# jabberjabberjabber/video-3d-pipeline

Measured on AMD Instinct MI355X. Metric: 1080p_sbs_to_4k_depth_frames_per_s, higher is better.
Workload: dtype int16 (SGM) + f64 (guided filter sums; f32 depth in/out)

## Files before the change

### video-3d-pipeline_amd/csrc/v3d_guided.hip

```cpp
#include "v3d_common.h"
#include <type_traits>

__device__ __forceinline__ double gf_rcp(double x)
{
    double r = __builtin_amdgcn_rcp(x);
    r = fma(r, fma(-x, r, 1.0), r);
    r = fma(r, fma(-x, r, 1.0), r);
    return r;
}

template <typename TD> __device__ __forceinline__ float gf_ld(const TD* p, size_t i);
template <> __device__ __forceinline__ float gf_ld<float>(const float* p, size_t i) { const float v = p[i]; return fabsf(v) <= 3.402823466e38f ? v : 0.f; }
template <> __device__ __forceinline__ float gf_ld<int16_t>(const int16_t* p, size_t i) { const int d = p[i]; return d > 0 ? (float)d * 0.0625f : 0.f; }
template <> __device__ __forceinline__ float gf_ld<uint16_t>(const uint16_t* p, size_t i) { return (float)p[i]; }

typedef unsigned short v3d_u16x2v __attribute__((ext_vector_type(2)));
typedef unsigned short v3d_u16x4 __attribute__((ext_vector_type(4)));
__device__ __forceinline__ void gf_st(float* p, float q) { *p = q; }
__device__ __forceinline__ void gf_st(uint16_t* p, float q) { *p = v3d_rint_u16(q); }

#define GF_TX 64
#define GF_RUN 8
#define GF_RMAX 16

template <typename TD>
__device__ __forceinline__ double gf_bilinear(const TD* __restrict__ src, int Ws, int Hs, double sx, double sy, int x, int y)
{
    const double fx = (x + 0.5) * sx - 0.5, fy = (y + 0.5) * sy - 0.5;
    const double x0f = floor(fx), y0f = floor(fy);
    const double wx = fx - x0f, wy = fy - y0f;
    const int x0 = (int)x0f, y0 = (int)y0f;
    const int xa = min(max(x0, 0), Ws - 1), xb = min(max(x0 + 1, 0), Ws - 1);
    const int ya = min(max(y0, 0), Hs - 1), yb = min(max(y0 + 1, 0), Hs - 1);
    const double top = (double)gf_ld(src, (size_t)ya * Ws + xa) * (1.0 - wx) + (double)gf_ld(src, (size_t)ya * Ws + xb) * wx;
    const double bot = (double)gf_ld(src, (size_t)yb * Ws + xa) * (1.0 - wx) + (double)gf_ld(src, (size_t)yb * Ws + xb) * wx;
    return top * (1.0 - wy) + bot * wy;
}

template <int SWEEP, int GF_RUNY, typename TD, typename TO>
__global__ __launch_bounds__(256) void k_gf(const TD* __restrict__ depth_lo, int Wlo, int Hlo,
                                            const uint8_t* __restrict__ guide, int W, int H, int r, double eps,
                                            double* __restrict__ A, double* __restrict__ B, TO* __restrict__ out)
{
    constexpr int NS = SWEEP == 1 ? 4 : 2;
    constexpr int GF_TY = 4 * GF_RUNY;
    extern __shared__ __attribute__((aligned(16))) double smem[];
    const int rows = GF_TY + 2 * r;
    const int pitch = (GF_TX + 2 * r) | 1;
    const int hp = GF_TX + 1;
    double* t0 = smem;
    double* t1 = t0 + rows * pitch;
    double* hs = t1 + rows * pitch;

    const int tid = threadIdx.x;
    const int ox = blockIdx.x * GF_TX, oy = blockIdx.y * GF_TY;
    const double sx = (double)Wlo / (double)W, sy = (double)Hlo / (double)H;

    const int tw = GF_TX + 2 * r;
    for (int i = tid; i < rows * tw; i += 256) {
        const int ty = i / tw, tx = i - ty * tw;
        const int gx = ox - r + tx, gy = oy - r + ty;
        double v0 = 0.0, v1 = 0.0;
        if (gx >= 0 && gx < W && gy >= 0 && gy < H) {
            if (SWEEP == 1) {
                v0 = (double)guide[(size_t)gy * W + gx] / 255.0;
                v1 = gf_bilinear(depth_lo, Wlo, Hlo, sx, sy, gx, gy);
            } else {
                v0 = A[(size_t)gy * W + gx];
                v1 = B[(size_t)gy * W + gx];
            }
        }
        t0[ty * pitch + tx] = v0;
        t1[ty * pitch + tx] = v1;
    }
    __syncthreads();

    const int nruns = GF_TX / GF_RUN;
    for (int task = tid; task < rows * nruns; task += 256) {
        const int row = task % rows, run = task / rows;
        const double* r0 = t0 + row * pitch + run * GF_RUN;
        const double* r1 = t1 + row * pitch + run * GF_RUN;
        double s0 = 0.0, s1 = 0.0, s2 = 0.0, s3 = 0.0;
        for (int k = 0; k <= 2 * r; k++) {
            const double u = r0[k], v = r1[k];
            s0 += u; s1 += v;
            if (SWEEP == 1) { s2 += u * u; s3 += u * v; }
        }
        double* h = hs + row * hp + run * GF_RUN;
        const int hplane = rows * hp;
        for (int j = 0; j < GF_RUN; j++) {
            h[j] = s0; h[hplane + j] = s1;
            if (SWEEP == 1) { h[2 * hplane + j] = s2; h[3 * hplane + j] = s3; }
            if (j + 1 < GF_RUN) {
                const double un = r0[j + 2 * r + 1], vn = r1[j + 2 * r + 1];
                const double uo = r0[j], vo = r1[j];
                s0 += un - uo; s1 += vn - vo;
                if (SWEEP == 1) { s2 += un * un - uo * uo; s3 += un * vn - uo * vo; }
            }
        }
    }
    __syncthreads();

    {
        const int x = tid % GF_TX, runy = tid / GF_TX;
        const int hplane = rows * hp;
        const double* h = hs + (runy * GF_RUNY) * hp + x;
        double s[NS];
#pragma unroll
        for (int q = 0; q < NS; q++) s[q] = 0.0;
        for (int k = 0; k <= 2 * r; k++)
#pragma unroll
            for (int q = 0; q < NS; q++) s[q] += h[q * hplane + k * hp];
        const int gx = ox + x;
        const int cx = min(gx + r, W - 1) - max(gx - r, 0) + 1;
        for (int j = 0; j < GF_RUNY; j++) {
            const int gy = oy + runy * GF_RUNY + j;
            if (gx < W && gy < H) {
                const int cy = min(gy + r, H - 1) - max(gy - r, 0) + 1;
                const double cnt = (double)(cx * cy);
                if (SWEEP == 1) {
                    const double mI = s[0] / cnt, mp = s[1] / cnt, mII = s[2] / cnt, mIp = s[3] / cnt;
                    const double var = mII - mI * mI, cov = mIp - mI * mp;
                    const double a = cov / (var + eps);
                    A[(size_t)gy * W + gx] = a;
                    B[(size_t)gy * W + gx] = mp - a * mI;
                } else {
                    const double I = (double)guide[(size_t)gy * W + gx] / 255.0;
                    const float q = (float)((s[0] / cnt) * I + (s[1] / cnt));
                    if constexpr (std::is_same<TO, float>::value) out[(size_t)gy * W + gx] = q;
                    else out[(size_t)gy * W + gx] = v3d_rint_u16(q);
                }
            }
            if (j + 1 < GF_RUNY) {
                const int kn = j + 2 * r + 1;
#pragma unroll
                for (int q = 0; q < NS; q++) s[q] += h[q * hplane + kn * hp] - h[q * hplane + j * hp];
            }
        }
    }
}

#ifndef GF_CH
#define GF_CH 3
#endif
typedef double v3d_f64x2 __attribute__((ext_vector_type(2)));
typedef float v3d_f32x2 __attribute__((ext_vector_type(2)));
typedef float v3d_f32x4 __attribute__((ext_vector_type(4)));

template <int SWEEP, int RR, typename TD, typename TO>
__global__ __launch_bounds__(256) void k_gfm(const TD* __restrict__ depth_lo, int Wlo, int Hlo,
                                             const uint8_t* __restrict__ guide, int W, int H, double eps, int band_h,
                                             double* __restrict__ A, double* __restrict__ B, TO* __restrict__ out,
                                             size_t depth_stride, size_t guide_stride)
{
    static_assert(RR % 2 == 0, "pairs must not straddle the strip's halo boundary");
    constexpr int R = 2 * RR + 1, NOUT = 256 - 2 * RR;
    __shared__ __attribute__((aligned(16))) double sVd[2][2][2][256];
    __shared__ __attribute__((aligned(16))) int2 sVi[2][2][256];
    {
        const size_t f = blockIdx.z, n4 = (size_t)W * H;
        depth_lo += f * depth_stride; guide += f * guide_stride; A += f * 2 * n4; B += f * 2 * n4; out += f * n4;
    }
    const int tid = threadIdx.x;
    const int gx = blockIdx.x * NOUT - RR + tid;
    const int ya = blockIdx.y * band_h, yb = min(ya + band_h, H);
    const bool col_ok = gx >= 0 && gx < W;
    const double sx = (double)Wlo / (double)W, sy = (double)Hlo / (double)H;
    const int nsteps = (yb - ya) + 2 * RR;

    const int hrow = tid >> 7, hq = tid & 127;
    const int hgx = blockIdx.x * NOUT - RR + 2 * hq;
    const bool pair_in = 2 * hq >= RR && 2 * hq < 256 - RR;
    const bool px0 = pair_in && hgx < W, px1 = pair_in && hgx + 1 < W;
    const bool vec_ok = px1 && (W & 1) == 0;

    int bxa = 0, bxb = 0; double bwx = 0.0;
    if (SWEEP == 1) {
        const double fx = (gx + 0.5) * sx - 0.5, x0f = floor(fx);
        bwx = fx - x0f;
        bxa = min(max((int)x0f, 0), Wlo - 1); bxb = min(max((int)x0f + 1, 0), Wlo - 1);
    }
    double r0[R], r1[R], v0 = 0.0, v1 = 0.0;
    int rg[R], vg = 0, vgg = 0;
#pragma unroll
    for (int j = 0; j < R; j++) { r0[j] = 0.0; r1[j] = 0.0; rg[j] = 0; }

    struct RowIn { int g; float a0, a1, b0, b1; double n0, n1; bool in; };
    const int gxc = min(max(gx, 0), W - 1);
    auto fetch_row = [&](int t) -> RowIn {
        RowIn q; q.g = 0; q.a0 = q.a1 = q.b0 = q.b1 = 0.f; q.n0 = q.n1 = 0.0;
        const int e = ya - RR + t;
        q.in = col_ok && e >= 0 && e < H && t < nsteps;
        const size_t o = (size_t)min(max(e, 0), H - 1) * W + gxc;
        if (SWEEP == 1) {
            q.g = guide[o];
            const double fy = (e + 0.5) * sy - 0.5, y0f = floor(fy);
            const TD* ra = depth_lo + (size_t)min(max((int)y0f, 0), Hlo - 1) * Wlo;
            const TD* rb = depth_lo + (size_t)min(max((int)y0f + 1, 0), Hlo - 1) * Wlo;
            q.a0 = gf_ld(ra, bxa); q.a1 = gf_ld(ra, bxb); q.b0 = gf_ld(rb, bxa); q.b1 = gf_ld(rb, bxb);
        } else {
            q.n0 = __builtin_nontemporal_load(A + o); q.n1 = __builtin_nontemporal_load(B + o);
        }
        return q;
    };
    RowIn nx[2] = { fetch_row(0), fetch_row(1) };

    int buf = 0;
    for (int t0 = 0; t0 < nsteps; t0 += 2 * R) {
#pragma unroll
        for (int s = 0; s < R; s++) {
            const int tA = t0 + 2 * s;
            if (tA < nsteps) {
                const int y0 = ya - 2 * RR + tA;
                const bool emit = y0 >= ya;
                const RowIn cur[2] = { nx[0], nx[1] };
                nx[0] = fetch_row(tA + 2); nx[1] = fetch_row(tA + 3);
#pragma unroll
                for (int rr = 0; rr < 2; rr++) {
                    const int j = (2 * s + rr) % R;
                    if (SWEEP == 1) {
                        int gn = 0; double pn = 0.0;
                        if (cur[rr].in) {
                            gn = cur[rr].g;
                            const int e = ya - RR + tA + rr;
                            const double fy = (e + 0.5) * sy - 0.5, wy = fy - floor(fy);
                            const double a0 = (double)cur[rr].a0, b0 = (double)cur[rr].b0;
                            const double top = fma(bwx, (double)cur[rr].a1 - a0, a0);
                            const double bot = fma(bwx, (double)cur[rr].b1 - b0, b0);
                            pn = fma(wy, bot - top, top);
                        }
                        const int go = rg[j]; const double po = r1[j];
                        rg[j] = gn; r1[j] = pn;
                        vg += gn - go; vgg += gn * gn - go * go;
                        v0 += pn - po; v1 = fma((double)gn, pn, fma(-(double)go, po, v1));
                    } else {
                        const double n0 = cur[rr].in ? cur[rr].n0 : 0.0, n1 = cur[rr].in ? cur[rr].n1 : 0.0;
                        const double o0 = r0[j], o1 = r1[j];
                        r0[j] = n0; r1[j] = n1;
                        v0 += n0 - o0; v1 += n1 - o1;
                    }
                    if (emit) {
                        sVd[buf][rr][0][tid] = v0; sVd[buf][rr][1][tid] = v1;
                        if (SWEEP == 1) sVi[buf][rr][tid] = make_int2(vg, vgg);
                    }
                }
                if (emit) {
                    __syncthreads();
                    const int y = y0 + hrow;
                    if (px0 && y < yb) {
                        double fq[2], lq[2], cq[2];
#pragma unroll
                        for (int q = 0; q < 2; q++) {
                            const v3d_f64x2* d = reinterpret_cast<const v3d_f64x2*>(&sVd[buf][hrow][q][0]) + (hq - RR / 2);
                            double f = 0.0, l = 0.0, c = 0.0;
#pragma unroll
                            for (int ch = 0; ch <= RR; ch += GF_CH) {
                                v3d_f64x2 w[GF_CH];
#pragma unroll
                                for (int i = 0; i < GF_CH; i++) if (ch + i <= RR) w[i] = d[ch + i];
#pragma unroll
                                for (int i = 0; i < GF_CH; i++) if (ch + i <= RR) {
                                    if (ch + i == 0) { f = w[i].x; c = w[i].y; }
                                    else if (ch + i == RR) { c += w[i].x; l = w[i].y; }
                                    else { c += w[i].x; c += w[i].y; }
                                }
                                asm volatile("" : "+v"(c) :: "memory");
                            }
                            fq[q] = f; lq[q] = l; cq[q] = c;
                        }
                        int g0 = 0, gg0 = 0, gl = 0, ggl = 0, cg = 0, cgg = 0;
                        if (SWEEP == 1) {
                            const int4* gi = reinterpret_cast<const int4*>(&sVi[buf][hrow][0]) + (hq - RR / 2);
#pragma unroll
                            for (int ch = 0; ch <= RR; ch += 3) {
                                int4 u[3];
#pragma unroll
                                for (int i = 0; i < 3; i++) if (ch + i <= RR) u[i] = gi[ch + i];
#pragma unroll
                                for (int i = 0; i < 3; i++) if (ch + i <= RR) {
                                    if (ch + i == 0) { g0 = u[i].x; gg0 = u[i].y; cg = u[i].z; cgg = u[i].w; }
                                    else if (ch + i == RR) { cg += u[i].x; cgg += u[i].y; gl = u[i].z; ggl = u[i].w; }
                                    else { cg += u[i].x + u[i].z; cgg += u[i].y + u[i].w; }
                                }
                                asm volatile("" : "+v"(cg), "+v"(cgg) :: "memory");
                            }
                        }
                        const double s0a = cq[0] + fq[0], s0b = cq[0] + lq[0], s1a = cq[1] + fq[1], s1b = cq[1] + lq[1];
                        const int cy = min(y + RR, H - 1) - max(y - RR, 0) + 1;
                        const int cx0 = min(hgx + RR, W - 1) - max(hgx - RR, 0) + 1, cx1 = min(hgx + 1 + RR, W - 1) - max(hgx + 1 - RR, 0) + 1;
                        const double inva = gf_rcp((double)(cx0 * cy)), invb = cx1 == cx0 ? inva : gf_rcp((double)(cx1 * cy));
                        const size_t o = (size_t)y * W + hgx;
                        if (SWEEP == 1) {
                            const int sga = cg + g0, sgb = cg + gl, sgga = cgg + gg0, sggb = cgg + ggl;
                            double ab[2][2];
#pragma unroll
                            for (int n = 0; n < 2; n++) {
                                const double inv = n ? invb : inva;
                                const double mI = (double)(n ? sgb : sga) * (inv * (1.0 / 255.0)), mp = (n ? s0b : s0a) * inv;
                                const double mII = (double)(n ? sggb : sgga) * (inv * (1.0 / 65025.0)), mIp = (n ? s1b : s1a) * (inv * (1.0 / 255.0));
                                const double var = fma(-mI, mI, mII), cov = fma(-mI, mp, mIp);
                                const double a = cov * gf_rcp(var + eps);
                                ab[n][0] = a; ab[n][1] = fma(-a, mI, mp);
                            }
                            if (vec_ok) {
                                v3d_f64x2 va = { ab[0][0], ab[1][0] }, vb = { ab[0][1], ab[1][1] };
                                __builtin_nontemporal_store(va, reinterpret_cast<v3d_f64x2*>(A + o));
                                __builtin_nontemporal_store(vb, reinterpret_cast<v3d_f64x2*>(B + o));
                            } else {
                                A[o] = ab[0][0]; B[o] = ab[0][1];
                                if (px1) { A[o + 1] = ab[1][0]; B[o + 1] = ab[1][1]; }
                            }
                        } else {
                            const double Ia = (double)guide[o] * (1.0 / 255.0);
                            const double Ib = px1 ? (double)guide[o + 1] * (1.0 / 255.0) : 0.0;
                            const float qa = (float)((s0a * inva) * Ia + (s1a * inva)), qb = (float)((s0b * invb) * Ib + (s1b * invb));
                            if (vec_ok && (std::is_same<TO, float>::value || (reinterpret_cast<uintptr_t>(out + o) & 3) == 0)) {
                                if constexpr (std::is_same<TO, float>::value) {
                                    v3d_f32x2 vq = { qa, qb };
                                    __builtin_nontemporal_store(vq, reinterpret_cast<v3d_f32x2*>(out + o));
                                } else {
                                    v3d_u16x2v vq = { v3d_rint_u16(qa), v3d_rint_u16(qb) };
                                    __builtin_nontemporal_store(vq, reinterpret_cast<v3d_u16x2v*>(out + o));
                                }
                            } else {
                                gf_st(out + o, qa);
                                if (px1) gf_st(out + o + 1, qb);
                            }
                        }
                    }
                    buf ^= 1;
                }
            }
        }
    }
}

__device__ __forceinline__ int gf_swz2(int m) { return m ^ ((m >> 3) & 1) ^ ((m >> 4) & 1); }
__device__ __forceinline__ int gf_swz4(int m) { return m ^ ((m >> 4) & 3); }
__device__ __forceinline__ int gf_c8(int c) { return 2 * gf_swz2(c >> 1) + (c & 1); }

template <int RR>
__device__ __forceinline__ void gf_run4(const double* row, int c0, double s[4])
{
    const v3d_f64x2* d = reinterpret_cast<const v3d_f64x2*>(row);
    const int m0 = (c0 - RR) >> 1;
    double c = 0.0, l0 = 0.0, l1 = 0.0, l2 = 0.0, r1 = 0.0, r2 = 0.0, r3 = 0.0;
#pragma unroll
    for (int k0 = 0; k0 < RR + 2; k0 += GF_CH) {
        v3d_f64x2 w[GF_CH];
#pragma unroll
        for (int i = 0; i < GF_CH; i++) if (k0 + i < RR + 2) w[i] = d[gf_swz2(m0 + k0 + i)];
#pragma unroll
        for (int i = 0; i < GF_CH; i++) {
            const int k = k0 + i;
            if (k == 0) { l0 = w[i].x; l1 = w[i].y; c = w[i].x; c += w[i].y; }
            else if (k == 1) { l2 = w[i].x; c += w[i].x; c += w[i].y; }
            else if (k < RR) { c += w[i].x; c += w[i].y; }
            else if (k == RR) { c += w[i].x; r1 = w[i].y; }
            else if (k == RR + 1) { r2 = w[i].x; r3 = w[i].y; }
        }
        asm volatile("" : "+v"(c) :: "memory");
    }
    s[0] = c; s[1] = (s[0] + r1) - l0; s[2] = (s[1] + r2) - l1; s[3] = (s[2] + r3) - l2;
}

template <int RR>
__device__ __forceinline__ void gf_run4(const int2* row, int c0, int2 s[4])
{
    const int4* d = reinterpret_cast<const int4*>(row);
    const int m0 = (c0 - RR) >> 1;
    int2 c = make_int2(0, 0), l0 = c, l1 = c, l2 = c, r1 = c, r2 = c, r3 = c;
#pragma unroll
    for (int k0 = 0; k0 < RR + 2; k0 += 3) {
        int4 w[3];
#pragma unroll
        for (int i = 0; i < 3; i++) if (k0 + i < RR + 2) w[i] = d[gf_swz2(m0 + k0 + i)];
#pragma unroll
        for (int i = 0; i < 3; i++) {
            const int k = k0 + i;
            const int2 a = make_int2(w[i].x, w[i].y), b = make_int2(w[i].z, w[i].w);
            if (k == 0) { l0 = a; l1 = b; c = make_int2(a.x + b.x, a.y + b.y); }
            else if (k == 1) { l2 = a; c.x += a.x + b.x; c.y += a.y + b.y; }
            else if (k < RR) { c.x += a.x + b.x; c.y += a.y + b.y; }
            else if (k == RR) { c.x += a.x; c.y += a.y; r1 = b; }
            else if (k == RR + 1) { r2 = a; r3 = b; }
        }
        asm volatile("" : "+v"(c.x), "+v"(c.y) :: "memory");
    }
    s[0] = c;
    s[1] = make_int2(s[0].x + r1.x - l0.x, s[0].y + r1.y - l0.y);
    s[2] = make_int2(s[1].x + r2.x - l1.x, s[1].y + r2.y - l1.y);
    s[3] = make_int2(s[2].x + r3.x - l2.x, s[2].y + r3.y - l2.y);
}

template <int RR>
__device__ __forceinline__ void gf_run4(const int4* row, int c0, int4 s[4])
{
    int4 c = make_int4(0, 0, 0, 0), l0 = c, l1 = c, l2 = c, r1 = c, r2 = c, r3 = c;
#pragma unroll
    for (int k0 = 0; k0 < 2 * RR + 4; k0 += 3) {
        int4 u[3];
#pragma unroll
        for (int i = 0; i < 3; i++) if (k0 + i < 2 * RR + 4) u[i] = row[gf_swz4(c0 - RR + k0 + i)];
#pragma unroll
        for (int i = 0; i < 3; i++) {
            const int k = k0 + i;
            if (k < 2 * RR + 1) { c.x += u[i].x; c.y += u[i].y; c.z += u[i].z; c.w += u[i].w; }
            if (k == 0) l0 = u[i];
            else if (k == 1) l1 = u[i];
            else if (k == 2) l2 = u[i];
            else if (k == 2 * RR + 1) r1 = u[i];
            else if (k == 2 * RR + 2) r2 = u[i];
            else if (k == 2 * RR + 3) r3 = u[i];
        }
        asm volatile("" : "+v"(c.x), "+v"(c.y), "+v"(c.z), "+v"(c.w) :: "memory");
    }
    s[0] = c;
    s[1] = make_int4(s[0].x - l0.x + r1.x, s[0].y - l0.y + r1.y, s[0].z - l0.z + r1.z, s[0].w - l0.w + r1.w);
    s[2] = make_int4(s[1].x - l1.x + r2.x, s[1].y - l1.y + r2.y, s[1].z - l1.z + r2.z, s[1].w - l1.w + r2.w);
    s[3] = make_int4(s[2].x - l2.x + r3.x, s[2].y - l2.y + r3.y, s[2].z - l2.z + r3.z, s[2].w - l2.w + r3.w);
}

template <int RR>
__device__ __forceinline__ void gf_solve4(const int sg[4], const int sgg[4], const double sp[4], const double sgp[4], int hgx, int y,
                                          int W, int H, double eps, double a[4], double b[4])
{
    const int cy = min(y + RR, H - 1) - max(y - RR, 0) + 1;
    int cx[4];
#pragma unroll
    for (int n = 0; n < 4; n++) cx[n] = min(hgx + n + RR, W - 1) - max(hgx + n - RR, 0) + 1;
    const double inv0 = gf_rcp((double)(cx[0] * cy));
#pragma unroll
    for (int n = 0; n < 4; n++) {
        const double inv = (n == 0 || cx[n] == cx[0]) ? inv0 : gf_rcp((double)(cx[n] * cy));
        const double mI = (double)sg[n] * (inv * (1.0 / 255.0)), mp = sp[n] * inv;
        const double mII = (double)sgg[n] * (inv * (1.0 / 65025.0)), mIp = sgp[n] * (inv * (1.0 / 255.0));
        const double var = fma(-mI, mI, mII), cov = fma(-mI, mp, mIp);
        const double aa = cov * gf_rcp(var + eps);
        a[n] = aa; b[n] = fma(-aa, mI, mp);
    }
}

template <int RR, int COLS, typename TD, bool I1, typename TO>
__global__ __launch_bounds__(2 * COLS, I1 ? 4 : 2) void k_gff(const TD* __restrict__ depth_lo, int Wlo, int Hlo,
                                                const uint8_t* __restrict__ guide, int W, int H, double eps, int band_h,
                                                TO* __restrict__ out, size_t depth_stride, size_t guide_stride)
{
    static_assert(RR % 4 == 0, "runs of four must not straddle the strip's halo boundaries");
    static_assert(!I1 || std::is_same<TD, int16_t>::value, "the integer stage 1 takes the int16 disparity");
    static_assert(COLS == 256 || (COLS == 512 && I1), "strip width (512 columns: I1 only, the f64 route's rows exceed the LDS)");
    constexpr int R = 2 * RR + 1, NOUT = COLS - 4 * RR, HR = COLS / 4;
    constexpr int S1D = 2 * 4 * 2 * COLS * 8, S1 = I1 ? 2 * 4 * COLS * 16 : S1D + 2 * 4 * COLS * 8;
    __shared__ __attribute__((aligned(16))) unsigned char sS1[S1];
    double (*sV1)[4][2][COLS] = reinterpret_cast<double (*)[4][2][COLS]>(sS1);
    int2 (*sVi)[4][COLS] = reinterpret_cast<int2 (*)[4][COLS]>(sS1 + (I1 ? 0 : S1D));
    int4 (*sVq)[4][COLS] = reinterpret_cast<int4 (*)[4][COLS]>(sS1);
    (void)sV1; (void)sVi; (void)sVq;
    __shared__ __attribute__((aligned(16))) double sAB[3][4][2][COLS];
    {
        const size_t f = blockIdx.z, n4 = (size_t)W * H;
        depth_lo += f * depth_stride; guide += f * guide_stride; out += f * n4;
    }
    const int role = __builtin_amdgcn_readfirstlane((int)(threadIdx.x / COLS));
    const int t = threadIdx.x % COLS;
    const int gx0 = blockIdx.x * NOUT - 2 * RR;
    const int gx = gx0 + t;
    const int ya = blockIdx.y * band_h, yb = min(ya + band_h, H);
    const int nrows = (yb - ya) + 4 * RR;
    const int NS = (nrows + 3) >> 2;
    const int NP = NS + 3;

    if (role == 0) {
        const bool col_ok = gx >= 0 && gx < W;
        const int gxc = min(max(gx, 0), W - 1);
        uint32_t ring[R];
        double r1[I1 ? 1 : R];
        uint32_t rgw[I1 ? 1 : (R + 3) / 4];
        int vg = 0, vgg = 0, vP = 0, vgP = 0;
        double v0 = 0.0, v1 = 0.0;
#pragma unroll
        for (int j = 0; j < R; j++) ring[j] = 0u;
#pragma unroll
        for (int j = 0; j < (I1 ? 1 : R); j++) r1[j] = 0.0;
#pragma unroll
        for (int j = 0; j < (I1 ? 1 : (R + 3) / 4); j++) rgw[j] = 0u;
        (void)ring; (void)r1; (void)rgw;
        int bxa, bxb, wxa = 0, wxb = 0; double bwx = 0.0;
        const double sx = (double)Wlo / (double)W, sy = (double)Hlo / (double)H;
        if constexpr (I1) {
            const int kx = gx >> 1;
            bxa = min(max((gx & 1) ? kx : kx - 1, 0), Wlo - 1); bxb = min(max((gx & 1) ? kx + 1 : kx, 0), Wlo - 1);
            wxa = (gx & 1) ? 3 : 1; wxb = 4 - wxa;
        } else {
            const double fx = (gx + 0.5) * sx - 0.5, x0f = floor(fx);
            bwx = fx - x0f;
            bxa = min(max((int)x0f, 0), Wlo - 1); bxb = min(max((int)x0f + 1, 0), Wlo - 1);
        }
        (void)wxa; (void)wxb; (void)bwx;
        struct RowIn { int g; typename std::conditional<I1, int, float>::type a0, a1, b0, b1; bool in; };
        auto fetch_row = [&](int tt) -> RowIn {
            RowIn q;
            const int e = ya - 2 * RR + tt;
            q.in = col_ok && e >= 0 && e < H && tt < nrows;
            const int ec = min(max(e, 0), H - 1);
            q.g = guide[(size_t)ec * W + gxc];
            if constexpr (I1) {
                const int ky = ec >> 1;
                const TD* ra = depth_lo + (size_t)min(max((ec & 1) ? ky : ky - 1, 0), Hlo - 1) * Wlo;
                const TD* rb = depth_lo + (size_t)min(max((ec & 1) ? ky + 1 : ky, 0), Hlo - 1) * Wlo;
                q.a0 = max((int)ra[bxa], 0); q.a1 = max((int)ra[bxb], 0); q.b0 = max((int)rb[bxa], 0); q.b1 = max((int)rb[bxb], 0);
            } else {
                const double fy = (e + 0.5) * sy - 0.5, y0f = floor(fy);
                const TD* ra = depth_lo + (size_t)min(max((int)y0f, 0), Hlo - 1) * Wlo;
                const TD* rb = depth_lo + (size_t)min(max((int)y0f + 1, 0), Hlo - 1) * Wlo;
                q.a0 = gf_ld(ra, bxa); q.a1 = gf_ld(ra, bxb); q.b0 = gf_ld(rb, bxa); q.b1 = gf_ld(rb, bxb);
            }
            return q;
        };
        RowIn nx[4] = { fetch_row(0), fetch_row(1), fetch_row(2), fetch_row(3) };
        for (int p0 = 0; p0 < NP; p0 += R) {
#pragma clang loop unroll(full)
            for (int sp = 0; sp < R; sp++) {
                const int p = p0 + sp;
                if (p < NP) {
                    int tl = t;
                    asm volatile("" : "+v"(tl));
                    const int hrow = tl / HR, c0 = 4 * (tl % HR), hgx = gx0 + c0;
                    const int j = p - 1;
                    if (j >= RR / 2 && j < NS) {
                        const int y = ya - 3 * RR + 4 * j + hrow;
                        double a[4] = { 0.0, 0.0, 0.0, 0.0 }, b[4] = { 0.0, 0.0, 0.0, 0.0 };
                        if (c0 >= RR && c0 < COLS - RR && y >= 0 && y < H && hgx >= 0 && hgx < W) {
                            int sg[4], sgg[4]; double sp_[4], sgp[4];
                            if constexpr (I1) {
                                int4 s[4];
                                gf_run4<RR>(&sVq[j & 1][hrow][0], c0, s);
#pragma unroll
                                for (int n = 0; n < 4; n++) {
                                    sg[n] = s[n].x; sgg[n] = s[n].y;
                                    sp_[n] = (double)s[n].z * (1.0 / 256.0); sgp[n] = (double)s[n].w * (1.0 / 256.0);
                                }
                            } else {
                                int2 si[4];
                                gf_run4<RR>(&sVi[j & 1][hrow][0], c0, si);
                                gf_run4<RR>(&sV1[j & 1][hrow][0][0], c0, sp_);
                                gf_run4<RR>(&sV1[j & 1][hrow][1][0], c0, sgp);
#pragma unroll
                                for (int n = 0; n < 4; n++) { sg[n] = si[n].x; sgg[n] = si[n].y; }
                            }
                            gf_solve4<RR>(sg, sgg, sp_, sgp, hgx, y, W, H, eps, a, b);
#pragma unroll
                            for (int n = 0; n < 4; n++) if (hgx + n >= W) { a[n] = 0.0; b[n] = 0.0; }
                        }
                        double* ab = &sAB[j % 3][hrow][0][0];
                        const int e0 = 2 * gf_swz2(c0 >> 1), e1 = 2 * gf_swz2((c0 >> 1) + 1);
                        *reinterpret_cast<v3d_f64x2*>(ab + e0) = v3d_f64x2{ a[0], a[1] };
                        *reinterpret_cast<v3d_f64x2*>(ab + e1) = v3d_f64x2{ a[2], a[3] };
                        *reinterpret_cast<v3d_f64x2*>(ab + COLS + e0) = v3d_f64x2{ b[0], b[1] };
                        *reinterpret_cast<v3d_f64x2*>(ab + COLS + e1) = v3d_f64x2{ b[2], b[3] };
                    }
                    if (p < NS) {
                        const int tA = 4 * p;
                        const RowIn cur[4] = { nx[0], nx[1], nx[2], nx[3] };
#pragma unroll
                        for (int k = 0; k < 4; k++) nx[k] = fetch_row(tA + 4 + k);
                        const bool emit = p >= RR / 2;
#pragma unroll
                        for (int rr = 0; rr < 4; rr++) {
                            const int slot = (4 * sp + rr) % R;
                            const int e = ya - 2 * RR + tA + rr;
                            if constexpr (I1) {
                                int gn = 0, Pn = 0;
                                if (cur[rr].in) {
                                    gn = cur[rr].g;
                                    const int wya = (e & 1) ? 3 : 1;
                                    Pn = wya * (wxa * cur[rr].a0 + wxb * cur[rr].a1) + (4 - wya) * (wxa * cur[rr].b0 + wxb * cur[rr].b1);
                                }
                                const int go = (int)(ring[slot] & 0xFFu), Po = (int)(ring[slot] >> 8);
                                ring[slot] = ((uint32_t)Pn << 8) | (uint32_t)gn;
                                vg += gn - go; vgg += gn * gn - go * go;
                                vP += Pn - Po; vgP += gn * Pn - go * Po;
                                if (emit) sVq[p & 1][rr][gf_swz4(t)] = make_int4(vg, vgg, vP, vgP);
                            } else {
                                int gn = 0; double pn = 0.0;
                                if (cur[rr].in) {
                                    gn = cur[rr].g;
                                    const double fy = (e + 0.5) * sy - 0.5, wy = fy - floor(fy);
                                    const double a0 = (double)cur[rr].a0, b0 = (double)cur[rr].b0;
                                    const double top = fma(bwx, (double)cur[rr].a1 - a0, a0);
                                    const double bot = fma(bwx, (double)cur[rr].b1 - b0, b0);
                                    pn = fma(wy, bot - top, top);
                                }
                                const int go = (int)((rgw[slot >> 2] >> (8 * (slot & 3))) & 0xFFu); const double po = r1[slot];
                                rgw[slot >> 2] = (rgw[slot >> 2] & ~(0xFFu << (8 * (slot & 3)))) | ((uint32_t)gn << (8 * (slot & 3)));
                                r1[slot] = pn;
                                vg += gn - go; vgg += gn * gn - go * go;
                                v0 += pn - po; v1 = fma((double)gn, pn, fma(-(double)go, po, v1));
                                if (emit) {
                                    const int ct = gf_c8(t);
                                    sV1[p & 1][rr][0][ct] = v0; sV1[p & 1][rr][1][ct] = v1;
                                    sVi[p & 1][rr][ct] = make_int2(vg, vgg);
                                }
                            }
                        }
                    }
                    __syncthreads();
                }
            }
        }
    } else {
        double r0[R], r1[R], va = 0.0, vb = 0.0;
#pragma unroll
        for (int j = 0; j < R; j++) { r0[j] = 0.0; r1[j] = 0.0; }
        for (int p0 = 0; p0 < NP; p0 += R) {
#pragma clang loop unroll(full)
            for (int sp = 0; sp < R; sp++) {
                const int p = p0 + sp;
                if (p < NP) {
                    int tl = t;
                    asm volatile("" : "+v"(tl));
                    const int hrow = tl / HR, c0 = 4 * (tl % HR), hgx = gx0 + c0;
                    {
                        const int j = p - 3;
                        const int y = ya - 4 * RR + 4 * j + hrow;
                        if (j >= RR && j < NS && c0 >= 2 * RR && c0 < COLS - 2 * RR && hgx < W && y < yb) {
                            double sa[4], sb[4];
                            gf_run4<RR>(&sAB[j % 3][hrow][0][0], c0, sa);
                            gf_run4<RR>(&sAB[j % 3][hrow][1][0], c0, sb);
                            const int cy = min(y + RR, H - 1) - max(y - RR, 0) + 1;
                            int cx[4];
#pragma unroll
                            for (int n = 0; n < 4; n++) cx[n] = min(hgx + n + RR, W - 1) - max(hgx + n - RR, 0) + 1;
                            const double inv0 = gf_rcp((double)(cx[0] * cy));
                            const size_t o = (size_t)y * W + hgx;
                            const bool all_in = hgx + 3 < W;
                            const bool vec_ok = all_in && (W & 3) == 0 && ((reinterpret_cast<uintptr_t>(out + o) | reinterpret_cast<uintptr_t>(guide + o)) & 3) == 0
                                                && (reinterpret_cast<uintptr_t>(out + o) & (4 * sizeof(TO) - 1)) == 0;
                            int g[4];
                            if (vec_ok) {
                                const uint32_t g4 = *reinterpret_cast<const uint32_t*>(guide + o);
#pragma unroll
                                for (int n = 0; n < 4; n++) g[n] = (g4 >> (8 * n)) & 0xFF;
                            } else {
#pragma unroll
                                for (int n = 0; n < 4; n++) g[n] = hgx + n < W ? guide[o + n] : 0;
                            }
                            float q[4];
#pragma unroll
                            for (int n = 0; n < 4; n++) {
                                const double inv = (n == 0 || cx[n] == cx[0]) ? inv0 : gf_rcp((double)(cx[n] * cy));
                                const double I = (double)g[n] * (1.0 / 255.0);
                                q[n] = (float)((sa[n] * inv) * I + (sb[n] * inv));
                            }
                            if (vec_ok) {
                                if constexpr (std::is_same<TO, float>::value) {
                                    const v3d_f32x4 vq = { q[0], q[1], q[2], q[3] };
                                    __builtin_nontemporal_store(vq, reinterpret_cast<v3d_f32x4*>(out + o));
                                } else {
                                    const v3d_u16x4 vq = { v3d_rint_u16(q[0]), v3d_rint_u16(q[1]), v3d_rint_u16(q[2]), v3d_rint_u16(q[3]) };
                                    __builtin_nontemporal_store(vq, reinterpret_cast<v3d_u16x4*>(out + o));
                                }
                            } else {
#pragma unroll
                                for (int n = 0; n < 4; n++) if (hgx + n < W) gf_st(out + o + n, q[n]);
                            }
                        }
                    }
                    {
                        const int j = p - 2;
                        if (j >= RR / 2 && j < NS) {
                            const bool emit = j >= RR;
                            double* col = &sAB[j % 3][0][0][gf_c8(tl)];
#pragma unroll
                            for (int rr = 0; rr < 4; rr++) {
                                const int slot = (4 * sp + rr) % R;
                                const double n0 = col[rr * 2 * COLS], n1 = col[rr * 2 * COLS + COLS];
                                const double o0 = r0[slot], o1 = r1[slot];
                                r0[slot] = n0; r1[slot] = n1;
                                va += n0 - o0; vb += n1 - o1;
                                if (emit) { col[rr * 2 * COLS] = va; col[rr * 2 * COLS + COLS] = vb; }
                            }
                        }
                    }
                    __syncthreads();
                }
            }
        }
    }
}

template <int RR, typename TD, typename TO>
static void launch_gff(const TD* depth_lo, int Wlo, int Hlo, const uint8_t* guide, int W, int H, double eps,
                       TO* out, int n, size_t depth_stride, size_t guide_stride, hipStream_t st)
{
    bool i1 = false;
    if constexpr (std::is_same<TD, int16_t>::value) i1 = g_v3d_opt.gf_int1 && W == 2 * Wlo && H == 2 * Hlo;
    const int cols = g_v3d_opt.gf_cols == 512 && i1 ? 512 : 256;
    int band = g_v3d_opt.gf_band;
    if (band <= 0) {
        int dev = 0, ncu = 256;
        (void)hipGetDevice(&dev);
        (void)hipDeviceGetAttribute(&ncu, hipDeviceAttributeMultiprocessorCount, dev);
        const long slots = (long)ncu * (cols == 256 && i1 ? 2 : 1), strips = v3d_cdiv(W, cols - 4 * RR);
        long best = -1;
        for (int nb = 1; nb <= 64 && nb <= H; nb++) {
            const int b = (v3d_cdiv(H, nb) + 1) & ~1;
            const long wgs = strips * v3d_cdiv(H, b) * n, rounds = (wgs + slots - 1) / slots, cost = rounds * (b + 4 * RR);
            if (best < 0 || cost < best) { best = cost; band = b; }
        }
    }
    const dim3 grid(v3d_cdiv(W, cols - 4 * RR), v3d_cdiv(H, band), n);
    if constexpr (std::is_same<TD, int16_t>::value) {
        if (i1 && cols == 512) {
            hipLaunchKernelGGL((k_gff<RR, 512, TD, true, TO>), grid, dim3(1024), 0, st, depth_lo, Wlo, Hlo, guide, W, H, eps, band, out, depth_stride, guide_stride);
            return;
        }
        if (i1) {
            hipLaunchKernelGGL((k_gff<RR, 256, TD, true, TO>), grid, dim3(512), 0, st, depth_lo, Wlo, Hlo, guide, W, H, eps, band, out, depth_stride, guide_stride);
            return;
        }
    }
    hipLaunchKernelGGL((k_gff<RR, 256, TD, false, TO>), grid, dim3(512), 0, st, depth_lo, Wlo, Hlo, guide, W, H, eps, band, out, depth_stride, guide_stride);
}

template <int RR, typename TD, typename TO>
static void launch_gfm(const TD* depth_lo, int Wlo, int Hlo, const uint8_t* guide, int W, int H, double eps,
                       double* A, double* B, TO* out, int n, size_t depth_stride, size_t guide_stride, hipStream_t st)
{
    const int band1 = g_v3d_opt.gf_band1, band2 = g_v3d_opt.gf_band2;
    const dim3 grid1(v3d_cdiv(W, 256 - 2 * RR), v3d_cdiv(H, band1), n), grid2(v3d_cdiv(W, 256 - 2 * RR), v3d_cdiv(H, band2), n);
    hipLaunchKernelGGL((k_gfm<1, RR, TD, TO>), grid1, dim3(256), 0, st, depth_lo, Wlo, Hlo, guide, W, H, eps, band1, A, B, out, depth_stride, guide_stride);
    hipLaunchKernelGGL((k_gfm<2, RR, TD, TO>), grid2, dim3(256), 0, st, depth_lo, Wlo, Hlo, guide, W, H, eps, band2, A, B, out, depth_stride, guide_stride);
}

extern "C" size_t v3d_guided_upscale_ws_bytes(int W, int H)
{
    if (W < 1 || H < 1) return 0;
    return (size_t)W * H * sizeof(double) * 2;
}

static size_t gf_smem(int r, int ns, int ty)
{
    const int rows = ty + 2 * r;
    const int pitch = (GF_TX + 2 * r) | 1;
    return sizeof(double) * ((size_t)2 * rows * pitch + (size_t)ns * rows * (GF_TX + 1));
}

template <typename TD, typename TO>
static int guided_upscale_batch(const TD* depth_lo, int Wlo, int Hlo, size_t depth_stride, const uint8_t* guide,
                                int W, int H, size_t guide_stride, int n, int r, float eps, TO* out, void* ws, void* stream)
{
    if (n < 1) { v3d_set_error("bad batch"); return V3D_ERR_ARG; }
    if (!depth_lo || !guide || !out || !ws) { v3d_set_error("null pointer"); return V3D_ERR_ARG; }
    if (Wlo < 1 || Hlo < 1 || W < 1 || H < 1) { v3d_set_error("bad geometry"); return V3D_ERR_ARG; }
    if (r < 1 || r > GF_RMAX) { v3d_set_error("radius %d outside [1, %d]", r, GF_RMAX); return V3D_ERR_UNSUPPORTED; }
    if (!(eps >= 0.f)) { v3d_set_error("eps must be >= 0"); return V3D_ERR_ARG; }
    if (((uintptr_t)ws & 15) != 0) { v3d_set_error("workspace must be 16-byte aligned"); return V3D_ERR_ARG; }
    hipStream_t st = (hipStream_t)stream;
    double* A = reinterpret_cast<double*>(ws);
    double* B = A + (size_t)W * H;
    if (!g_v3d_opt.gf_tiled && g_v3d_opt.gf_fused && (r == 4 || r == 8)) {
        if (r == 4) launch_gff<4>(depth_lo, Wlo, Hlo, guide, W, H, (double)eps, out, n, depth_stride, guide_stride, st);
        else launch_gff<8>(depth_lo, Wlo, Hlo, guide, W, H, (double)eps, out, n, depth_stride, guide_stride, st);
        V3D_LAUNCH_CHECK();
        return V3D_OK;
    }
    if (!g_v3d_opt.gf_tiled && (r == 4 || r == 8)) {
        if (r == 4) launch_gfm<4>(depth_lo, Wlo, Hlo, guide, W, H, (double)eps, A, B, out, n, depth_stride, guide_stride, st);
        else launch_gfm<8>(depth_lo, Wlo, Hlo, guide, W, H, (double)eps, A, B, out, n, depth_stride, guide_stride, st);
        V3D_LAUNCH_CHECK();
        return V3D_OK;
    }
    for (int f = 0; f < n; f++) {
    const TD* depth_lo_f = depth_lo + (size_t)f * depth_stride; const uint8_t* guide_f = guide + (size_t)f * guide_stride;
    double* A = reinterpret_cast<double*>(ws) + (size_t)f * 2 * W * H; double* B = A + (size_t)W * H; TO* out_f = out + (size_t)f * W * H;
    const int ty = r <= 8 ? 16 : 8;
    const dim3 grid(v3d_cdiv(W, GF_TX), v3d_cdiv(H, ty));
    const size_t sm1 = gf_smem(r, 4, ty), sm2 = gf_smem(r, 2, ty);
    if (ty == 16) {
        V3D_HIP_CHECK(hipFuncSetAttribute((const void*)k_gf<1, 4, TD, TO>, hipFuncAttributeMaxDynamicSharedMemorySize, (int)sm1));
        V3D_HIP_CHECK(hipFuncSetAttribute((const void*)k_gf<2, 4, TD, TO>, hipFuncAttributeMaxDynamicSharedMemorySize, (int)sm2));
        hipLaunchKernelGGL((k_gf<1, 4, TD, TO>), grid, dim3(256), sm1, st, depth_lo_f, Wlo, Hlo, guide_f, W, H, r, (double)eps, A, B, out_f);
        hipLaunchKernelGGL((k_gf<2, 4, TD, TO>), grid, dim3(256), sm2, st, depth_lo_f, Wlo, Hlo, guide_f, W, H, r, (double)eps, A, B, out_f);
    } else {
        V3D_HIP_CHECK(hipFuncSetAttribute((const void*)k_gf<1, 2, TD, TO>, hipFuncAttributeMaxDynamicSharedMemorySize, (int)sm1));
        V3D_HIP_CHECK(hipFuncSetAttribute((const void*)k_gf<2, 2, TD, TO>, hipFuncAttributeMaxDynamicSharedMemorySize, (int)sm2));
        hipLaunchKernelGGL((k_gf<1, 2, TD, TO>), grid, dim3(256), sm1, st, depth_lo_f, Wlo, Hlo, guide_f, W, H, r, (double)eps, A, B, out_f);
        hipLaunchKernelGGL((k_gf<2, 2, TD, TO>), grid, dim3(256), sm2, st, depth_lo_f, Wlo, Hlo, guide_f, W, H, r, (double)eps, A, B, out_f);
    }
    }
    V3D_LAUNCH_CHECK();
    return V3D_OK;
}

extern "C" int v3d_guided_upscale_batch(const float* depth_lo, int Wlo, int Hlo, size_t depth_stride, const uint8_t* guide,
                                        int W, int H, size_t guide_stride, int n, int r, float eps, float* out, void* ws, void* stream)
{
    return guided_upscale_batch<float, float>(depth_lo, Wlo, Hlo, depth_stride, guide, W, H, guide_stride, n, r, eps, out, ws, stream);
}

extern "C" int v3d_guided_upscale(const float* depth_lo, int Wlo, int Hlo, const uint8_t* guide, int W, int H,
                                  int r, float eps, float* out, void* ws, void* stream)
{
    return guided_upscale_batch<float, float>(depth_lo, Wlo, Hlo, 0, guide, W, H, 0, 1, r, eps, out, ws, stream);
}

extern "C" int v3d_guided_upscale_disp16_batch(const int16_t* disp16, int Wlo, int Hlo, size_t disp_stride, const uint8_t* guide,
                                               int W, int H, size_t guide_stride, int n, int r, float eps, float* out, void* ws, void* stream)
{
    return guided_upscale_batch<int16_t, float>(disp16, Wlo, Hlo, disp_stride, guide, W, H, guide_stride, n, r, eps, out, ws, stream);
}

extern "C" int v3d_guided_upscale_u16_batch(const uint16_t* depth_lo, int Wlo, int Hlo, size_t depth_stride, const uint8_t* guide,
                                            int W, int H, size_t guide_stride, int n, int r, float eps, uint16_t* out, void* ws, void* stream)
{
    return guided_upscale_batch<uint16_t, uint16_t>(depth_lo, Wlo, Hlo, depth_stride, guide, W, H, guide_stride, n, r, eps, out, ws, stream);
}
```

Measured before the change: 2612.

## Use raw LDS addressing and buffer loads in guided filter kernel

Rewrites the LDS box-sum readers to compute swizzled addresses directly as raw LDS byte offsets with XOR pairing, which needs the shared arrays aligned to 1024 bytes. The integer stage-1 path fetches four guide rows and four low-res depth rows per step through buffer loads with out-of-bounds handling, and shares the vertical interpolation across the four output rows. It also uses 24-bit multiplies and branchless bounds tests. This cuts address arithmetic and redundant global loads, at the cost of dependence on the alignment and on a new 2^31-pixel guard for the integer path.

```diff
diff --git a/video-3d-pipeline_amd/csrc/v3d_guided.hip b/video-3d-pipeline_amd/csrc/v3d_guided.hip
--- a/video-3d-pipeline_amd/csrc/v3d_guided.hip
+++ b/video-3d-pipeline_amd/csrc/v3d_guided.hip
@@ -339,19 +339,30 @@
 __device__ __forceinline__ int gf_swz4(int m) { return m ^ ((m >> 4) & 3); }
 __device__ __forceinline__ int gf_c8(int c) { return 2 * gf_swz2(c >> 1) + (c & 1); }
 
+#define GF_ROW_ALIGN 1024
+typedef int gf_i32x4 __attribute__((ext_vector_type(4)));
+typedef __attribute__((address_space(3))) const v3d_f64x2 gf_lds_f64x2;
+typedef __attribute__((address_space(3))) const gf_i32x4 gf_lds_i32x4;
+__device__ __forceinline__ uint32_t gf_lds_addr(const void* p) { return (uint32_t)(uintptr_t)(__attribute__((address_space(3))) const void*)p; }
+__device__ __forceinline__ uint32_t gf_pair_addr(uint32_t w0, int jp) { const uint32_t w = w0 + 32u * jp; return w | (((w >> 3) ^ (w >> 4)) & 16u); }
+__device__ __forceinline__ uint32_t gf_quad_addr(uint32_t w0, int jg) { const uint32_t w = w0 + 64u * jg; return w | ((w >> 4) & 48u); }
+
 template <int RR>
-__device__ __forceinline__ void gf_run4(const double* row, int c0, double s[4])
-{
-    const v3d_f64x2* d = reinterpret_cast<const v3d_f64x2*>(row);
-    const int m0 = (c0 - RR) >> 1;
+__device__ __forceinline__ void gf_run4(const double* row, int c0, double s[4], uint32_t plane = 0u)
+{
+    static_assert(RR % 4 == 0, "aligned pairs of chunks, read as 4 + 4 + 2 (r = 8) or 4 + 2 (r = 4)");
+    const uint32_t w0 = gf_lds_addr(row) + 8u * (uint32_t)(c0 - RR);
     double c = 0.0, l0 = 0.0, l1 = 0.0, l2 = 0.0, r1 = 0.0, r2 = 0.0, r3 = 0.0;
 #pragma unroll
-    for (int k0 = 0; k0 < RR + 2; k0 += GF_CH) {
-        v3d_f64x2 w[GF_CH];
-#pragma unroll
-        for (int i = 0; i < GF_CH; i++) if (k0 + i < RR + 2) w[i] = d[gf_swz2(m0 + k0 + i)];
-#pragma unroll
-        for (int i = 0; i < GF_CH; i++) {
+    for (int k0 = 0; k0 < RR + 2; k0 += 4) {
+        v3d_f64x2 w[4];
+#pragma unroll
+        for (int i = 0; i < 4; i += 2) if (k0 + i < RR + 2) {
+            const uint32_t a = gf_pair_addr(w0, (k0 + i) / 2);
+            w[i] = *(gf_lds_f64x2*)(uintptr_t)(a + plane); w[i + 1] = *(gf_lds_f64x2*)(uintptr_t)((a ^ 16u) + plane);
+        }
+#pragma unroll
+        for (int i = 0; i < 4; i++) {
             const int k = k0 + i;
             if (k == 0) { l0 = w[i].x; l1 = w[i].y; c = w[i].x; c += w[i].y; }
             else if (k == 1) { l2 = w[i].x; c += w[i].x; c += w[i].y; }
@@ -367,16 +378,18 @@
 template <int RR>
 __device__ __forceinline__ void gf_run4(const int2* row, int c0, int2 s[4])
 {
-    const int4* d = reinterpret_cast<const int4*>(row);
-    const int m0 = (c0 - RR) >> 1;
+    const uint32_t w0 = gf_lds_addr(row) + 8u * (uint32_t)(c0 - RR);
     int2 c = make_int2(0, 0), l0 = c, l1 = c, l2 = c, r1 = c, r2 = c, r3 = c;
 #pragma unroll
-    for (int k0 = 0; k0 < RR + 2; k0 += 3) {
-        int4 w[3];
-#pragma unroll
-        for (int i = 0; i < 3; i++) if (k0 + i < RR + 2) w[i] = d[gf_swz2(m0 + k0 + i)];
-#pragma unroll
-        for (int i = 0; i < 3; i++) {
+    for (int k0 = 0; k0 < RR + 2; k0 += 4) {
+        gf_i32x4 w[4];
+#pragma unroll
+        for (int i = 0; i < 4; i += 2) if (k0 + i < RR + 2) {
+            const uint32_t a = gf_pair_addr(w0, (k0 + i) / 2);
+            w[i] = *(gf_lds_i32x4*)(uintptr_t)a; w[i + 1] = *(gf_lds_i32x4*)(uintptr_t)(a ^ 16u);
+        }
+#pragma unroll
+        for (int i = 0; i < 4; i++) {
             const int k = k0 + i;
             const int2 a = make_int2(w[i].x, w[i].y), b = make_int2(w[i].z, w[i].w);
             if (k == 0) { l0 = a; l1 = b; c = make_int2(a.x + b.x, a.y + b.y); }
@@ -396,16 +409,18 @@
 template <int RR>
 __device__ __forceinline__ void gf_run4(const int4* row, int c0, int4 s[4])
 {
-    int4 c = make_int4(0, 0, 0, 0), l0 = c, l1 = c, l2 = c, r1 = c, r2 = c, r3 = c;
-#pragma unroll
-    for (int k0 = 0; k0 < 2 * RR + 4; k0 += 3) {
-        int4 u[3];
-#pragma unroll
-        for (int i = 0; i < 3; i++) if (k0 + i < 2 * RR + 4) u[i] = row[gf_swz4(c0 - RR + k0 + i)];
-#pragma unroll
-        for (int i = 0; i < 3; i++) {
+    const uint32_t w0 = gf_lds_addr(row) + 16u * (uint32_t)(c0 - RR);
+    gf_i32x4 c = { 0, 0, 0, 0 }, l0 = c, l1 = c, l2 = c, r1 = c, r2 = c, r3 = c;
+#pragma unroll
+    for (int k0 = 0; k0 < 2 * RR + 4; k0 += 4) {
+        const uint32_t a = gf_quad_addr(w0, k0 / 4);
+        gf_i32x4 u[4];
+#pragma unroll
+        for (int i = 0; i < 4; i++) u[i] = *(gf_lds_i32x4*)(uintptr_t)(a ^ (16u * i));
+#pragma unroll
+        for (int i = 0; i < 4; i++) {
             const int k = k0 + i;
-            if (k < 2 * RR + 1) { c.x += u[i].x; c.y += u[i].y; c.z += u[i].z; c.w += u[i].w; }
+            if (k < 2 * RR + 1) c += u[i];
             if (k == 0) l0 = u[i];
             else if (k == 1) l1 = u[i];
             else if (k == 2) l2 = u[i];
@@ -413,12 +428,11 @@
             else if (k == 2 * RR + 2) r2 = u[i];
             else if (k == 2 * RR + 3) r3 = u[i];
         }
-        asm volatile("" : "+v"(c.x), "+v"(c.y), "+v"(c.z), "+v"(c.w) :: "memory");
-    }
-    s[0] = c;
-    s[1] = make_int4(s[0].x - l0.x + r1.x, s[0].y - l0.y + r1.y, s[0].z - l0.z + r1.z, s[0].w - l0.w + r1.w);
-    s[2] = make_int4(s[1].x - l1.x + r2.x, s[1].y - l1.y + r2.y, s[1].z - l1.z + r2.z, s[1].w - l1.w + r2.w);
-    s[3] = make_int4(s[2].x - l2.x + r3.x, s[2].y - l2.y + r3.y, s[2].z - l2.z + r3.z, s[2].w - l2.w + r3.w);
+        asm volatile("" : "+v"(c) :: "memory");
+    }
+    const gf_i32x4 s1 = c - l0 + r1, s2 = s1 - l1 + r2, s3 = s2 - l2 + r3;
+    s[0] = make_int4(c.x, c.y, c.z, c.w); s[1] = make_int4(s1.x, s1.y, s1.z, s1.w);
+    s[2] = make_int4(s2.x, s2.y, s2.z, s2.w); s[3] = make_int4(s3.x, s3.y, s3.z, s3.w);
 }
 
 template <int RR>
@@ -429,10 +443,10 @@
     int cx[4];
 #pragma unroll
     for (int n = 0; n < 4; n++) cx[n] = min(hgx + n + RR, W - 1) - max(hgx + n - RR, 0) + 1;
-    const double inv0 = gf_rcp((double)(cx[0] * cy));
+    const double inv0 = gf_rcp((double)(int)__umul24((uint32_t)cx[0], (uint32_t)cy));
 #pragma unroll
     for (int n = 0; n < 4; n++) {
-        const double inv = (n == 0 || cx[n] == cx[0]) ? inv0 : gf_rcp((double)(cx[n] * cy));
+        const double inv = (n == 0 || cx[n] == cx[0]) ? inv0 : gf_rcp((double)(int)__umul24((uint32_t)cx[n], (uint32_t)cy));
         const double mI = (double)sg[n] * (inv * (1.0 / 255.0)), mp = sp[n] * inv;
         const double mII = (double)sgg[n] * (inv * (1.0 / 65025.0)), mIp = sgp[n] * (inv * (1.0 / 255.0));
         const double var = fma(-mI, mI, mII), cov = fma(-mI, mp, mIp);
@@ -451,12 +465,13 @@
     static_assert(COLS == 256 || (COLS == 512 && I1), "strip width (512 columns: I1 only, the f64 route's rows exceed the LDS)");
     constexpr int R = 2 * RR + 1, NOUT = COLS - 4 * RR, HR = COLS / 4;
     constexpr int S1D = 2 * 4 * 2 * COLS * 8, S1 = I1 ? 2 * 4 * COLS * 16 : S1D + 2 * 4 * COLS * 8;
-    __shared__ __attribute__((aligned(16))) unsigned char sS1[S1];
+    static_assert((COLS * 8) % 512 == 0 && (COLS * 16) % GF_ROW_ALIGN == 0 && S1D % GF_ROW_ALIGN == 0, "row alignment of the swizzled LDS rows");
+    __shared__ __attribute__((aligned(GF_ROW_ALIGN))) unsigned char sS1[S1];
     double (*sV1)[4][2][COLS] = reinterpret_cast<double (*)[4][2][COLS]>(sS1);
     int2 (*sVi)[4][COLS] = reinterpret_cast<int2 (*)[4][COLS]>(sS1 + (I1 ? 0 : S1D));
     int4 (*sVq)[4][COLS] = reinterpret_cast<int4 (*)[4][COLS]>(sS1);
     (void)sV1; (void)sVi; (void)sVq;
-    __shared__ __attribute__((aligned(16))) double sAB[3][4][2][COLS];
+    __shared__ __attribute__((aligned(GF_ROW_ALIGN))) double sAB[3][4][2][COLS];
     {
         const size_t f = blockIdx.z, n4 = (size_t)W * H;
         depth_lo += f * depth_stride; guide += f * guide_stride; out += f * n4;
@@ -497,27 +512,48 @@
             bxa = min(max((int)x0f, 0), Wlo - 1); bxb = min(max((int)x0f + 1, 0), Wlo - 1);
         }
         (void)wxa; (void)wxb; (void)bwx;
-        struct RowIn { int g; typename std::conditional<I1, int, float>::type a0, a1, b0, b1; bool in; };
-        auto fetch_row = [&](int tt) -> RowIn {
-            RowIn q;
-            const int e = ya - 2 * RR + tt;
-            q.in = col_ok && e >= 0 && e < H && tt < nrows;
-            const int ec = min(max(e, 0), H - 1);
-            q.g = guide[(size_t)ec * W + gxc];
-            if constexpr (I1) {
-                const int ky = ec >> 1;
-                const TD* ra = depth_lo + (size_t)min(max((ec & 1) ? ky : ky - 1, 0), Hlo - 1) * Wlo;
-                const TD* rb = depth_lo + (size_t)min(max((ec & 1) ? ky + 1 : ky, 0), Hlo - 1) * Wlo;
-                q.a0 = max((int)ra[bxa], 0); q.a1 = max((int)ra[bxb], 0); q.b0 = max((int)rb[bxa], 0); q.b1 = max((int)rb[bxb], 0);
-            } else {
+        struct StepIn { int16_t d[4][2]; uint8_t g[4]; };
+        const __amdgpu_buffer_rsrc_t rs_d = buf_rsrc(depth_lo, (uint32_t)Wlo * (uint32_t)Hlo * 2u), rs_g = buf_rsrc(guide, (uint32_t)W * (uint32_t)H);
+        const uint32_t og = col_ok ? (uint32_t)gxc : V3D_BUF_OOB;
+        const uint32_t oa = col_ok ? 2u * (uint32_t)bxa : V3D_BUF_OOB, ob = col_ok ? 2u * (uint32_t)bxb : V3D_BUF_OOB;
+        const int par = ya & 1;
+        auto fetch_step = [&](int s) -> StepIn {
+            StepIn q;
+            const int e0 = ya - 2 * RR + 4 * s, sb = (e0 >> 1) - 1 + par;
+#pragma unroll
+            for (int j = 0; j < 4; j++) {
+                const uint32_t so = (uint32_t)min(max(sb + j, 0), Hlo - 1) * (2u * (uint32_t)Wlo);
+                q.d[j][0] = __builtin_amdgcn_raw_buffer_load_b16(rs_d, oa, so, 0);
+                q.d[j][1] = __builtin_amdgcn_raw_buffer_load_b16(rs_d, ob, so, 0);
+            }
+#pragma unroll
+            for (int i = 0; i < 4; i++)
+                q.g[i] = __builtin_amdgcn_raw_buffer_load_b8(rs_g, og, (uint32_t)min(max(e0 + i, 0), H - 1) * (uint32_t)W, 0);
+            return q;
+        };
+        (void)rs_d; (void)rs_g; (void)og; (void)oa; (void)ob; (void)par;
+        struct RowIn { int g; float a0, a1, b0, b1; bool in; };
+        struct RowIn4 { RowIn r[4]; };
+        auto fetch_rows = [&](int t0) -> RowIn4 {
+            RowIn4 q4;
+#pragma unroll
+            for (int k = 0; k < 4; k++) {
+                RowIn& q = q4.r[k];
+                const int tt = t0 + k, e = ya - 2 * RR + tt;
+                q.in = col_ok && e >= 0 && e < H && tt < nrows;
+                const int ec = min(max(e, 0), H - 1);
+                q.g = guide[(size_t)ec * W + gxc];
                 const double fy = (e + 0.5) * sy - 0.5, y0f = floor(fy);
                 const TD* ra = depth_lo + (size_t)min(max((int)y0f, 0), Hlo - 1) * Wlo;
                 const TD* rb = depth_lo + (size_t)min(max((int)y0f + 1, 0), Hlo - 1) * Wlo;
                 q.a0 = gf_ld(ra, bxa); q.a1 = gf_ld(ra, bxb); q.b0 = gf_ld(rb, bxa); q.b1 = gf_ld(rb, bxb);
             }
-            return q;
+            return q4;
         };
-        RowIn nx[4] = { fetch_row(0), fetch_row(1), fetch_row(2), fetch_row(3) };
+        (void)fetch_step; (void)fetch_rows;
+        typename std::conditional<I1, StepIn, RowIn4>::type nxt;
+        if constexpr (I1) nxt = fetch_step(0);
+        else nxt = fetch_rows(0);
         for (int p0 = 0; p0 < NP; p0 += R) {
 #pragma clang loop unroll(full)
             for (int sp = 0; sp < R; sp++) {
@@ -530,7 +566,7 @@
                     if (j >= RR / 2 && j < NS) {
                         const int y = ya - 3 * RR + 4 * j + hrow;
                         double a[4] = { 0.0, 0.0, 0.0, 0.0 }, b[4] = { 0.0, 0.0, 0.0, 0.0 };
-                        if (c0 >= RR && c0 < COLS - RR && y >= 0 && y < H && hgx >= 0 && hgx < W) {
+                        if ((int)(c0 >= RR) & (int)(c0 < COLS - RR) & (int)(y >= 0) & (int)(y < H) & (int)(hgx >= 0) & (int)(hgx < W)) {
                             int sg[4], sgg[4]; double sp_[4], sgp[4];
                             if constexpr (I1) {
                                 int4 s[4];
@@ -544,13 +580,16 @@
                                 int2 si[4];
                                 gf_run4<RR>(&sVi[j & 1][hrow][0], c0, si);
                                 gf_run4<RR>(&sV1[j & 1][hrow][0][0], c0, sp_);
-                                gf_run4<RR>(&sV1[j & 1][hrow][1][0], c0, sgp);
+                                gf_run4<RR>(&sV1[j & 1][hrow][0][0], c0, sgp, COLS * 8u);
 #pragma unroll
                                 for (int n = 0; n < 4; n++) { sg[n] = si[n].x; sgg[n] = si[n].y; }
                             }
                             gf_solve4<RR>(sg, sgg, sp_, sgp, hgx, y, W, H, eps, a, b);
-#pragma unroll
-                            for (int n = 0; n < 4; n++) if (hgx + n >= W) { a[n] = 0.0; b[n] = 0.0; }
+                            if (hgx + 3 >= W) {
+                                asm volatile("");
+#pragma unroll
+                                for (int n = 1; n < 4; n++) if (hgx + n >= W) { a[n] = 0.0; b[n] = 0.0; }
+                            }
                         }
                         double* ab = &sAB[j % 3][hrow][0][0];
                         const int e0 = 2 * gf_swz2(c0 >> 1), e1 = 2 * gf_swz2((c0 >> 1) + 1);
@@ -561,34 +600,50 @@
                     }
                     if (p < NS) {
                         const int tA = 4 * p;
-                        const RowIn cur[4] = { nx[0], nx[1], nx[2], nx[3] };
-#pragma unroll
-                        for (int k = 0; k < 4; k++) nx[k] = fetch_row(tA + 4 + k);
                         const bool emit = p >= RR / 2;
-#pragma unroll
-                        for (int rr = 0; rr < 4; rr++) {
-                            const int slot = (4 * sp + rr) % R;
-                            const int e = ya - 2 * RR + tA + rr;
-                            if constexpr (I1) {
-                                int gn = 0, Pn = 0;
-                                if (cur[rr].in) {
-                                    gn = cur[rr].g;
-                                    const int wya = (e & 1) ? 3 : 1;
-                                    Pn = wya * (wxa * cur[rr].a0 + wxb * cur[rr].a1) + (4 - wya) * (wxa * cur[rr].b0 + wxb * cur[rr].b1);
+                        if constexpr (I1) {
+                            const StepIn cs = nxt;
+                            nxt = fetch_step(p + 1);
+                            uint32_t h[4], P4[4];
+#pragma unroll
+                            for (int j = 0; j < 4; j++)
+                                h[j] = __umul24((uint32_t)wxa, (uint32_t)max((int)cs.d[j][0], 0)) + __umul24((uint32_t)wxb, (uint32_t)max((int)cs.d[j][1], 0));
+                            P4[0] = __umul24(h[1], 3u) + h[0]; P4[1] = __umul24(h[1], 3u) + h[2];
+                            P4[2] = __umul24(h[2], 3u) + h[1]; P4[3] = __umul24(h[2], 3u) + h[3];
+                            if (par) {
+                                asm volatile("v_mov_b32 %3, %2\n\tv_mov_b32 %2, %1\n\tv_mov_b32 %1, %0"
+                                             : "+v"(P4[0]), "+v"(P4[1]), "+v"(P4[2]), "+v"(P4[3]));
+                                P4[0] = __umul24(h[0], 3u) + h[1];
+                            }
+#pragma unroll
+                            for (int rr = 0; rr < 4; rr++) {
+                                const int slot = (4 * sp + rr) % R;
+                                const int e = ya - 2 * RR + tA + rr;
+                                uint32_t gn = cs.g[rr], Pn = P4[rr];
+                                if (!(e >= 0 && e < H && tA + rr < nrows)) {
+                                    asm volatile("");
+                                    gn = 0u; Pn = 0u;
                                 }
-                                const int go = (int)(ring[slot] & 0xFFu), Po = (int)(ring[slot] >> 8);
-                                ring[slot] = ((uint32_t)Pn << 8) | (uint32_t)gn;
-                                vg += gn - go; vgg += gn * gn - go * go;
-                                vP += Pn - Po; vgP += gn * Pn - go * Po;
+                                const uint32_t go = ring[slot] & 0xFFu, Po = ring[slot] >> 8;
+                                ring[slot] = (Pn << 8) | gn;
+                                vg += (int)(gn - go); vgg += (int)(__umul24(gn, gn) - __umul24(go, go));
+                                vP += (int)(Pn - Po); vgP += (int)(__umul24(gn, Pn) - __umul24(go, Po));
                                 if (emit) sVq[p & 1][rr][gf_swz4(t)] = make_int4(vg, vgg, vP, vgP);
-                            } else {
+                            }
+                        } else {
+                            const RowIn4 cur = nxt;
+                            nxt = fetch_rows(tA + 4);
+#pragma unroll
+                            for (int rr = 0; rr < 4; rr++) {
+                                const int slot = (4 * sp + rr) % R;
+                                const int e = ya - 2 * RR + tA + rr;
                                 int gn = 0; double pn = 0.0;
-                                if (cur[rr].in) {
-                                    gn = cur[rr].g;
+                                if (cur.r[rr].in) {
+                                    gn = cur.r[rr].g;
                                     const double fy = (e + 0.5) * sy - 0.5, wy = fy - floor(fy);
-                                    const double a0 = (double)cur[rr].a0, b0 = (double)cur[rr].b0;
-                                    const double top = fma(bwx, (double)cur[rr].a1 - a0, a0);
-                                    const double bot = fma(bwx, (double)cur[rr].b1 - b0, b0);
+                                    const double a0 = (double)cur.r[rr].a0, b0 = (double)cur.r[rr].b0;
+                                    const double top = fma(bwx, (double)cur.r[rr].a1 - a0, a0);
+                                    const double bot = fma(bwx, (double)cur.r[rr].b1 - b0, b0);
                                     pn = fma(wy, bot - top, top);
                                 }
                                 const int go = (int)((rgw[slot >> 2] >> (8 * (slot & 3))) & 0xFFu); const double po = r1[slot];
@@ -626,12 +681,12 @@
                         if (j >= RR && j < NS && c0 >= 2 * RR && c0 < COLS - 2 * RR && hgx < W && y < yb) {
                             double sa[4], sb[4];
                             gf_run4<RR>(&sAB[j % 3][hrow][0][0], c0, sa);
-                            gf_run4<RR>(&sAB[j % 3][hrow][1][0], c0, sb);
+                            gf_run4<RR>(&sAB[j % 3][hrow][0][0], c0, sb, COLS * 8u);
                             const int cy = min(y + RR, H - 1) - max(y - RR, 0) + 1;
                             int cx[4];
 #pragma unroll
                             for (int n = 0; n < 4; n++) cx[n] = min(hgx + n + RR, W - 1) - max(hgx + n - RR, 0) + 1;
-                            const double inv0 = gf_rcp((double)(cx[0] * cy));
+                            const double inv0 = gf_rcp((double)(int)__umul24((uint32_t)cx[0], (uint32_t)cy));
                             const size_t o = (size_t)y * W + hgx;
                             const bool all_in = hgx + 3 < W;
                             const bool vec_ok = all_in && (W & 3) == 0 && ((reinterpret_cast<uintptr_t>(out + o) | reinterpret_cast<uintptr_t>(guide + o)) & 3) == 0
@@ -648,7 +703,7 @@
                             float q[4];
 #pragma unroll
                             for (int n = 0; n < 4; n++) {
-                                const double inv = (n == 0 || cx[n] == cx[0]) ? inv0 : gf_rcp((double)(cx[n] * cy));
+                                const double inv = (n == 0 || cx[n] == cx[0]) ? inv0 : gf_rcp((double)(int)__umul24((uint32_t)cx[n], (uint32_t)cy));
                                 const double I = (double)g[n] * (1.0 / 255.0);
                                 q[n] = (float)((sa[n] * inv) * I + (sb[n] * inv));
                             }
@@ -694,7 +749,7 @@
                        TO* out, int n, size_t depth_stride, size_t guide_stride, hipStream_t st)
 {
     bool i1 = false;
-    if constexpr (std::is_same<TD, int16_t>::value) i1 = g_v3d_opt.gf_int1 && W == 2 * Wlo && H == 2 * Hlo;
+    if constexpr (std::is_same<TD, int16_t>::value) i1 = g_v3d_opt.gf_int1 && W == 2 * Wlo && H == 2 * Hlo && (size_t)W * H < ((size_t)1 << 31);
     const int cols = g_v3d_opt.gf_cols == 512 && i1 ? 512 : 256;
     int band = g_v3d_opt.gf_band;
     if (band <= 0) {
```

New measurement: 2691 (median of 6 runs). +3.0%, better.
